# manasakani/DeviceKMC

Hardware: AMD Instinct MI355X
Metric: KMC steps/sec (higher is better)
Workload: dtype f64

## Files before the change

devicekmc_amd/csrc/common.h:

```cpp
#pragma once
#include <hip/hip_runtime.h>
#include <stdint.h>
#include <stdio.h>
#include <string.h>
#include <math.h>
#include "../../include/devicekmc_hip.h"
#include "../../include/devicekmc_hip_debug.h"

enum { DEFECT = 0, OXYGEN_DEFECT = 1, VACANCY = 2, O_EL = 3, Hf_EL = 4, Ni_EL = 5, Ti_EL = 6, Pt_EL = 7, N_EL = 8, NULL_ELEMENT = 9 };
enum { EV_GEN = 0, EV_REC = 1, EV_VDIFF = 2, EV_IDIFF = 3, EV_NULL = 4 };

#define DKMC_KB 8.617333262e-5
#define DKMC_Q 1.60217663e-19
#define DKMC_HBAR 1.054571817e-34
#define DKMC_MAX_LAYERS 5
#define WAVE 64

struct MetalSet { int n; const int *e; };

__device__ __forceinline__ bool is_metal(int el, const MetalSet &ms)
{
    bool r = false;
    for (int t = 0; t < ms.n; ++t) r |= (ms.e[t] == el);
    return r;
// ... 137 lines not shown
    double cg_tol = 1e-6;
    int current_warm_start = 1;
    int profiling = 0;
    int cb_edge_domain = 0;
    long long tcache_budget = -1;
    double pair_cut = 6.5;
    int pair_form = 0;
    int k_blocked = 1;
    int k_blocked_large = 0;
    int k_window_word_bytes = 4;
    int x_aux = 2;
    int x_slab = 1;
    int k_slab = 1;
    int x_poly = X_POLY_DEFAULT;
    int x_poly_auto = 1;
    int x_poly_rows[2] = {0, 0};
    int x_poly_form = 2;
    int x_poly1_degree = 0;
    int x_poly_form_used = 0, x_poly_products = 0;
    int x_stop_form = 2;
    double x_stop_margin = X_STOP_MARGIN_DEFAULT;
    XStopLast x_stop_last{};
    int x_slab_poly = 0;
    int x_aux_warm = 0;
    int x_items_kc = 0;
    int x_apply_form = 0;
    int x_tile_f32 = 1;
    double x_tile_drop = 0.0;
    int x_tile_drop_unit = 0;
    int x_tile_drop_auto = 1;
    long long x_tile_drop_gate = 0;
    double x_tile_drop_used = 0.0;
    int xtl_census_form = 1;
    int x_static_tiles = 2;
    int x_static_gate = 0;
    int x_static_nM = -1;
    int x_static_verify = 0;
    int x_tile_f32_fail_once = 0;
    int x_fold_form = 1;
    int x_fold_poison = 0;
    int x_nmul_form = 1;
    int x_nmul_lane_bytes = 16;
    int x_nmul_window = 2;
    int x_nmul_window_cap = 76 * 1024;
    int x_nmul_window_block = 320;
    int x_block = 16;
    int x_format = 1;
    int current_map = 0;
    int x_iter_hint = 0;
    int event_temperature = 0;
    int event_census = 0;
    int event_census_valid = 0;
    double event_census_info[16] = {0};
    dkmc_stats stats{};
    char err[512] = {0};
    int err_code = 0;
    double E_gen[DKMC_MAX_LAYERS] = {0}, E_rec[DKMC_MAX_LAYERS] = {0}, E_Vdiff[DKMC_MAX_LAYERS] = {0}, E_Odiff[DKMC_MAX_LAYERS] = {0};
    int num_layers = 0;
    static const int NBUF = 192;
    void *buf[NBUF] = {nullptr};
    size_t bufsz[NBUF] = {0};
};

constexpr int X_STATIC_GATE = 32768;
static inline int x_static_rule(int ns, int gate_override) { return ns >= (gate_override > 0 ? gate_override : X_STATIC_GATE) ? 1 : 0; }
Engine &eng();
// ... 70 lines not shown
```

devicekmc_amd/csrc/engine.hip:

```cpp
#include "common.h"
#include <stdlib.h>

int events_upload_layers();
void xstate_reset(const void *key);

static Engine g_engine;
Engine &eng() { return g_engine; }

int dkmc_fail(int code, const char *what, const char *file, int line)
{
    Engine &e = eng();
    snprintf(e.err, sizeof(e.err), "%s (%s:%d)", what, file, line);
    e.err_code = code ? code : -1;
    fprintf(stderr, "devicekmc_hip: %s\n", e.err);
    return e.err_code;
}

void *scratch(int slot, size_t bytes)
{
    Engine &e = eng();
    if (bytes == 0) bytes = 16;
    if (e.bufsz[slot] < bytes) {
        if (e.buf[slot]) { (void)hipStreamSynchronize(e.stream); (void)hipFree(e.buf[slot]); }
        size_t want = bytes + bytes / 8 + 256;
// ... 52 lines not shown
int dkmc_get_x_poly_form_used(void) { return eng().x_poly_form_used; }
int dkmc_get_x_poly_products(void) { return eng().x_poly_products; }
void dkmc_set_x_stop_form(int form) { eng().x_stop_form = form == 1 ? 1 : (form == 2 ? 2 : 0); }
int dkmc_get_x_stop_form(void) { return eng().x_stop_form; }
void dkmc_set_x_stop_margin(double kappa) { eng().x_stop_margin = (kappa > 0.0 && kappa <= 1.0) ? kappa : X_STOP_MARGIN_DEFAULT; }
double dkmc_get_x_stop_margin(void) { return eng().x_stop_margin; }
int dkmc_get_x_stop_info(int *fired, double *norm, double *rz, double *true_residual)
{
    const XStopLast &l = eng().x_stop_last;
    if (fired) *fired = l.fired;
    if (norm) *norm = l.norm;
    if (rz) *rz = l.rz;
    if (true_residual) *true_residual = l.true_res;
    return l.fired ? 0 : 1;
}
void dkmc_debug_set_x_poly1_degree(int n) { eng().x_poly1_degree = n < 0 ? 0 : (n > 20 ? 20 : n); }
void dkmc_set_x_poly_auto_rows(int n0, int n1) { Engine &e = eng(); e.x_poly_rows[0] = n0 > 0 ? n0 : 0; e.x_poly_rows[1] = n1 > e.x_poly_rows[0] ? n1 : e.x_poly_rows[0]; }
void dkmc_set_x_apply_form(int form) { eng().x_apply_form = form == 1 ? 1 : 0; }
int dkmc_get_x_apply_form(void) { return eng().x_apply_form; }
void dkmc_set_x_tile_f32(int mode) { eng().x_tile_f32 = mode == 0 ? 0 : 1; }
int dkmc_get_x_tile_f32(void) { return eng().x_tile_f32; }
void dkmc_set_x_tile_drop(double theta) { eng().x_tile_drop = theta > 0.0 ? (theta > 1e-4 ? 1e-4 : theta) : 0.0; }
double dkmc_get_x_tile_drop(void) { return eng().x_tile_drop; }
void dkmc_set_x_tile_drop_unit(int unit) { eng().x_tile_drop_unit = unit == 1 ? 1 : 0; }
int dkmc_get_x_tile_drop_unit(void) { return eng().x_tile_drop_unit; }
void dkmc_set_x_tile_drop_auto(int on) { eng().x_tile_drop_auto = on ? 1 : 0; }
int dkmc_get_x_tile_drop_auto(void) { return eng().x_tile_drop_auto; }
void dkmc_set_x_tile_drop_auto_subblocks(long long gate) { eng().x_tile_drop_gate = gate > 0 ? gate : 0; }
double dkmc_get_x_tile_drop_used(void) { return eng().x_tile_drop_used; }
void dkmc_debug_fail_true_residual_once(void) { eng().x_tile_f32_fail_once = 1; }
void dkmc_set_x_fold_form(int form) { eng().x_fold_form = form == 0 ? 0 : 1; }
int dkmc_get_x_fold_form(void) { return eng().x_fold_form; }
void dkmc_debug_poison_fold_cells(int on) { eng().x_fold_poison = on ? 1 : 0; }
void dkmc_set_x_static_tiles(int mode) { eng().x_static_tiles = (mode == 0 || mode == 1) ? mode : 2; }
int dkmc_get_x_static_tiles(void) { return eng().x_static_tiles; }
int dkmc_debug_x_static_verify(int on) { const int was = eng().x_static_verify; eng().x_static_verify = on ? 1 : 0; return was; }
void dkmc_debug_set_x_static_gate(int members) { eng().x_static_gate = members > 0 ? members : 0; }
int dkmc_x_static_rule(int members) { return x_static_rule(members, eng().x_static_gate); }
int dkmc_x_static_strips(int n_metals) { return n_metals > 0 ? n_metals / 256 : 0; }
void dkmc_set_x_nmul_form(int form) { eng().x_nmul_form = form == 0 ? 0 : 1; }
int dkmc_get_x_nmul_form(void) { return eng().x_nmul_form; }
void dkmc_set_x_nmul_lane_bytes(int bytes) { eng().x_nmul_lane_bytes = bytes == 8 ? 8 : 16; }
int dkmc_get_x_nmul_lane_bytes(void) { return eng().x_nmul_lane_bytes; }
void dkmc_set_x_nmul_window(int mode) { eng().x_nmul_window = (mode == 0 || mode == 1) ? mode : 2; }
int dkmc_get_x_nmul_window(void) { return eng().x_nmul_window; }
void dkmc_debug_set_x_nmul_window(int cap_bytes, int block_rows)
{
    Engine &e = eng();
    e.x_nmul_window_cap = cap_bytes < 0 ? 76 * 1024 : (cap_bytes > 76 * 1024 ? 76 * 1024 : cap_bytes);
    e.x_nmul_window_block = (block_rows >= 16 && block_rows <= 1024 && block_rows % 16 == 0) ? block_rows : 320;
}
void dkmc_set_x_slab(int on) { eng().x_slab = on ? 1 : 0; }
int dkmc_get_x_slab(void) { return eng().x_slab; }
void dkmc_set_x_slab_poly(int on) { eng().x_slab_poly = on ? 1 : 0; }
int dkmc_get_x_slab_poly(void) { return eng().x_slab_poly; }
void dkmc_set_x_block(int s) { eng().x_block = s < 1 ? 1 : (s > 16 ? 16 : s); }
int dkmc_get_x_block(void) { return eng().x_block; }
void dkmc_set_x_aux(int mode) { eng().x_aux = mode < 0 ? 0 : (mode > 3 ? 2 : mode); }
int dkmc_get_x_aux(void) { return eng().x_aux; }
void dkmc_set_k_blocked(int on) { eng().k_blocked = on ? 1 : 0; }
int dkmc_get_k_blocked(void) { return eng().k_blocked; }
void dkmc_set_k_blocked_large(int on) { eng().k_blocked_large = on ? 1 : 0; }
int dkmc_get_k_blocked_large(void) { return eng().k_blocked_large; }
void dkmc_set_k_window_word_bytes(int bytes) { eng().k_window_word_bytes = bytes == 2 ? 2 : 4; }
int dkmc_get_k_window_word_bytes(void) { return eng().k_window_word_bytes; }
void dkmc_set_cb_edge_domain(int atoms_only) { eng().cb_edge_domain = atoms_only ? 1 : 0; }
// ... 125 lines not shown
```

devicekmc_amd/csrc/xt.hip:

```cpp
#include "xtiles.h"
#include <hip/hip_ext.h>
int tc_prepare_tiled(const XParams &P, dkmc_gpubuf *buf, int ns, const SEntry *S, const int *aflag, const int *srank, const int *atom_site,
                     int c_lo, int c_hi, int sharded, TCacheView *out);
#include <vector>
#include <algorithm>
#include <stdlib.h>
#include <string.h>

__device__ __forceinline__ double xt_tvalue(const XParams &P, double prefac, const TCacheView &TC,
                                            double x1, double y1, double z1, double cb1, int f1, int slot1, int slotA1, int mr1,
                                            double x2, double y2, double z2, double cb2, int f2, int slot2, int slotA2, int mr2,
                                            bool have_pre = false, double pre = 0.0)
{
    const double d = site_dist(x1, y1, z1, x2, y2, z2, P.laty, P.latz, P.pbc);
    if (d < P.nn_dist) return 0.0;
    const int kind = tunnel_kind<AF_MP_VAL>(f1, f2, cb1, cb2, P.tol);
    if (!kind) return 0.0;
    if (kind == 1 && TC.enabled) {
        const bool v1 = f1 & AF_V;
        double cv;
        if (have_pre && !v1) { if (pre == pre) return -pre; }
        else if (tc_lookup(TC, v1 ? slot1 : slot2, v1 ? slotA1 : slotA2, v1 ? mr2 : mr1, cv)) return -cv;
    }
    return -wkb_T(kind, 1e-10 * d, fabs(cb1 - cb2), prefac, P.V0);
// ... 886 lines not shown

int xt_assemble_and_solve(dkmc_gpubuf *buf, const XParams &P, int ns, const SEntry *S, const int *aneigh, const int *ancnt, const int *aflag,
                          const int *srank, const int *atom_site, double *rhs, double *y, int *iters_out, double *rr_out, double *yaux, int yaux_valid, int warm)
{
    TCacheView TC{};
    Engine &e = eng(); hipStream_t st = e.stream;
    XTState &X = g_xt; X.valid = false;
    g_xlive = XLive{};
    const int Na = P.Na, Nsub = Na + 1;
    X.Nsub = Nsub; X.ns = ns;
    const int ns_pad = ((ns + XT_C - 1) / XT_C) * XT_C + XT_C;
    X.ns_pad = ns_pad;
    const int nK = (ns + XT_R - 1) / XT_R, nW = (ns + XT_C - 1) / XT_C;
    X.nK = nK; X.nW = nW;
    const long long ncell = (long long)nK * nW;
    if (ncell > 0x7ffffff0ll) return dkmc_fail(47, "update_power: too many tile cells", __FILE__, __LINE__);

    const int nbr = (Nsub + 255) / 256, m = Nsub;
    const bool sharded = comm_attached() != 0;
    const int nr = sharded ? comm_nranks() : 1, me = sharded ? comm_rank() : 0;
    int rc = 0, ntiles = 0;
    long long xs_nnz = 0;
    int *cnt = nullptr, *nsrank = nullptr, *col = nullptr, *si = nullptr, *srow = nullptr, *nitem_w = nullptr;
    xrp_t *rp = nullptr, *dpos = nullptr;
    double *val = nullptr, *sd = nullptr, *tval = nullptr, *rowpart = nullptr, *colpart = nullptr, *sc = nullptr, *r = nullptr, *p = nullptr, *t = nullptr,
           *q = nullptr, *vS = nullptr, *part = nullptr, *qS = nullptr, *sS = nullptr, *xS = nullptr, *part_pt = nullptr, *part_rr = nullptr;
    XTile *tiles = nullptr; int2 *wrange = nullptr; int *wlist = nullptr; XItem *items = nullptr; unsigned long long *d_cnt = nullptr; XCtrl *ctrl = nullptr;
    float *tval32 = nullptr;
    SNodes SN{};
    double *xbuf = nullptr;
    XStatic &K = g_xs;
    const bool k_had = K.valid;
    K.valid = false; K.pending = false; K.reused = false; K.verify_nnz = -1;
    const int nM_first = (!sharded && e.x_format != 0) ? e.x_static_nM : -1;
    const int w_static = nM_first >= 0 ? xs_w_static(nM_first) : 0;
    for (int c = 0; c < 8; ++c) K.info[c] = 0;
    for (int c = 0; c < 4; ++c) K.verify[c] = 0;
    K.info[0] = nM_first >= 0 ? 1 : 0; K.info[1] = w_static; K.info[6] = XS_NA; K.info[7] = -1;
    int t_static = 0, xs_reason = XS_NA; long long sub_static = 0;
    bool k_cand = false;
    auto assemble = [&]() -> int {
        if (g_fault_phase == 1) { g_fault_phase = 0; return dkmc_fail(90, "injected fault (assembly of X)", __FILE__, __LINE__); }
        if (sharded) { xbuf = (double *)scratch(S_CG_XCHG, ((size_t)ns * (e.x_block > 1 ? 16 : 1) + 2) * (e.x_block > 1 ? comm_nranks() : 1) * 8); if (!xbuf) return e.err_code; if (ns > 0) { rc = side_stream_init(g_side); if (rc) return rc; } }
        cnt = (int *)scratch(S_X_CNT, (size_t)(Nsub + 4) * 4);
        rp = (xrp_t *)scratch(S_X_ROWPTR, (size_t)(Nsub + 4) * sizeof(xrp_t));
        dpos = (xrp_t *)scratch(S_XT_DPOS, (size_t)(Nsub + 4) * sizeof(xrp_t));
        nsrank = (int *)scratch(S_X_SCB, (size_t)(Nsub + 4) * 4);
        if (!cnt || !rp || !dpos || !nsrank) return e.err_code;
        hipLaunchKernelGGL((k_xpat_plain<0>), dim3(nbr), dim3(256), 0, st, P, (const int *)nullptr, aneigh, ancnt, cnt, (const xrp_t *)nullptr, (int *)nullptr);
        rc = dkmc_exclusive_scan_i32_i64(cnt, rp, Nsub, rp + Nsub); if (rc) return rc;
        HIPCHK(hipMemcpyAsync(&xs_nnz, rp + Nsub, sizeof(long long), hipMemcpyDeviceToHost, st));
        HIPCHK(hipStreamSynchronize(st));
        if (xs_nnz <= 0) return dkmc_fail(10, "update_power: empty X", __FILE__, __LINE__);
        X.xs_nnz = xs_nnz;
        col = (int *)scratch(S_X_COL, (size_t)xs_nnz * 4);
        val = (double *)scratch(S_X_DATA, (size_t)xs_nnz * 8);
        if (!col || !val) return e.err_code;
        hipLaunchKernelGGL((k_xpat_plain<1>), dim3(nbr), dim3(256), 0, st, P, (const int *)nullptr, aneigh, ancnt, cnt, (const xrp_t *)rp, col);
        hipLaunchKernelGGL((k_xval<16>), dim3((Nsub + 15) / 16), dim3(256), 0, st, P, Nsub, (const SEntry *)nullptr, 0, (const int *)nullptr, (const xrp_t *)rp,
                           (const int *)col, (const double *)buf->atom_x, (const double *)buf->atom_y, (const double *)buf->atom_z, aflag,
                           (const double *)buf->atom_CB_edge, val, TCacheView{}, atom_site, dpos);
        hipLaunchKernelGGL(k_xt_node_srank, dim3(nbr), dim3(256), 0, st, Nsub, srank, nsrank);
        KCHK();
        g_xb.rp = rp; g_xb.dpos = dpos; g_xb.ci = col; g_xb.val = val; g_xb.nsrank = nsrank;
        g_xb.ax = buf->atom_x; g_xb.ay = buf->atom_y; g_xb.az = buf->atom_z;

// ... 110 lines not shown
                tval32 = (float *)scratch_try(S_XT_TVAL32, b32);
            }
            if (tval32) e.stats.x_tile_f32_bytes = (long long)b32; else e.stats.x_tile_stream = -1;
        }
        HIPCHK(hipMemsetAsync(rowpart, 0, (size_t)(ncell + 1) * XT_R * 8, st));
        HIPCHK(hipMemsetAsync(colpart, 0, (size_t)(X.nitems + 1) * XT_C * 8, st));
        HIPCHK(hipMemsetAsync(d_cnt, 0, 16, st));
        if (k_cand && (tval32 != nullptr) != K.img) { k_cand = false; xs_reason = XS_IMAGE; }
        if (w_static > 0 && !k_cand) { rc = xs_reserve(nM_first, t_static); if (rc) return rc; }
        const int t_fill0 = k_cand ? t_static : 0;
        if (nM_first < 0) {
            if (X.tile_n > 0)
                hipLaunchKernelGGL((k_xt_fill<0>), dim3(X.tile_n), dim3(XT_NT), 0, st, P, ns, (const XTile *)tiles + X.tile_lo, (int)X.sub_base, SN, TC, tval, d_cnt, tval32, 0);
        } else {
            if (t_fill0 == 0 && t_static > 0)
                hipLaunchKernelGGL((k_xt_fill<0>), dim3(t_static), dim3(XT_NT), 0, st, P, ns, (const XTile *)tiles, (int)X.sub_base, SN, TC, tval, d_cnt, tval32, t_static);
            if (X.tile_n - t_static > 0)
                hipLaunchKernelGGL((k_xt_fill<1>), dim3(X.tile_n - t_static), dim3(XT_NT), 0, st, P, ns, (const XTile *)tiles + t_static, (int)X.sub_base, SN, TC, tval, d_cnt, tval32, 0);
        }
        KCHK();
        K.info[2] = k_cand ? t_static : 0; K.info[3] = X.tile_n - t_fill0; K.info[4] = k_cand ? sub_static : 0; K.info[5] = X.sub_n - (k_cand ? sub_static : 0); K.info[6] = xs_reason;
        if (w_static > 0) {
            if (!k_cand) {
                if (t_static > 0) HIPCHK(hipMemcpyAsync(K.tiles, tiles, (size_t)t_static * sizeof(XTile), hipMemcpyDeviceToDevice, st));
                hipLaunchKernelGGL(k_xs_snapshot, dim3((nM_first + 255) / 256), dim3(256), 0, st, nM_first, SN, K.snap_d, K.snap_f);
                KCHK();
                const double par[6] = {P.tol, P.nn_dist, P.m_e, P.V0, P.laty, P.latz};
                memcpy(K.par, par, sizeof(par)); K.pbc = P.pbc;
                K.key = (const void *)buf->site_x; K.nM = nM_first; K.w_static = w_static; K.t_static = t_static; K.sub_static = sub_static;
            }
            K.tval = e.buf[S_XT_TVAL]; K.tval_cap = e.bufsz[S_XT_TVAL]; K.img = tval32 != nullptr;
            K.tval32 = K.img ? e.buf[S_XT_TVAL32] : nullptr; K.tval32_cap = K.img ? e.bufsz[S_XT_TVAL32] : 0;
            K.pending = true; K.reused = k_cand;
        }
        if (e.x_static_verify && nM_first >= 0 && ncell > 0) {
            rc = xs_verify(P, ns, nK, nW, ncell, SN, TC, cmask, tiles, ntiles, X.nsub_total, tval, tval32); if (rc) return rc;
        }
        g_xb.tval32 = tval32;
        g_xb.tval = tval; g_xb.rowpart = rowpart; g_xb.colpart = colpart;
        X.valid = true;

        sc = (double *)scratch(S_CG_S, (size_t)m * 8); r = (double *)scratch(S_CG_R, (size_t)m * 8);
        p = (double *)scratch(S_CG_P, (size_t)m * 8); t = (double *)scratch(S_CG_T, (size_t)m * 8);
        q = (double *)scratch(S_XT_Q, (size_t)m * 8);
        vS = (double *)scratch(S_CG_PS, (size_t)ns_pad * 3 * 8);
        part = (double *)scratch(S_CG_PART, (size_t)3 * 8192 * 8);
        ctrl = (XCtrl *)scratch(S_CG_CTRL, sizeof(XCtrl));
        if (!sc || !r || !p || !t || !q || !vS || !part || !ctrl) return e.err_code;
        qS = vS; sS = vS + ns_pad; xS = vS + 2 * (size_t)ns_pad;
        HIPCHK(hipMemsetAsync(vS, 0, (size_t)ns_pad * 3 * 8, st));
        part_pt = part; part_rr = part + 4096;
        return 0;
    };
    rc = assemble();
    if (sharded) rc = comm_agree(rc, "assembly of X");
    if (rc) return rc;

    const double tol2 = e.cg_tol * e.cg_tol;

    if (ns > 0) {
        hipLaunchKernelGGL(k_xt_fill_f64, dim3((ns + 255) / 256), dim3(256), 0, st, qS, (long long)ns, 1.0);
        rc = xt_tile_sums<0>(qS, xS, 1); if (rc) return rc;
    }
    hipLaunchKernelGGL(k_xt_scale_init, dim3(nbr), dim3(256), 0, st, m, (const xrp_t *)dpos, val, (const int *)nsrank, (const double *)xS, sc, rhs, y, q, sS, qS);
    KCHK();

// ... 484 lines not shown
```

devicekmc_amd/csrc/xt_live.h:

```cpp
#pragma once

XLive g_xlive;

constexpr double XTL_DROP_AUTO_THETA = 1e-10;
constexpr long long XTL_DROP_GATE = 246272;
double xtl_drop_rule(long long stored_subblocks, long long gate_override)
{
    const long long gate = gate_override > 0 ? gate_override : XTL_DROP_GATE;
    return stored_subblocks > 0 && stored_subblocks >= gate ? XTL_DROP_AUTO_THETA : 0.0;
}
extern "C" double dkmc_xtl_drop_rule(long long stored_subblocks) { return xtl_drop_rule(stored_subblocks, eng().x_tile_drop_gate); }

__global__ __launch_bounds__(XT_NT) void k_xtl_census(int nK, const XTile *__restrict__ tiles, int sub_base, const double *__restrict__ tval,
                                                      const double *__restrict__ sS, double theta, int unit, unsigned *__restrict__ lcmask,
                                                      int *__restrict__ tflag, unsigned long long *__restrict__ cnt)
{
    __shared__ double rs[XT_R], mx[XT_C / XT_SBW];
    const XTile td = tiles[blockIdx.x];
    const int tid = threadIdx.x, q = tid >> 5, c = tid & 31;
    if (tid < XT_R) rs[tid] = sS[XT_R * td.k + tid];
    __syncthreads();
    double m = 0.0;
    if ((td.mask >> q) & 1u) {
        const int sl = __popc(td.mask & ((1u << q) - 1u));
// ... 44 lines not shown
            const int r0 = 8 * (it >> 1) + 2 * (it & 1) + (l >> 4);
            const double ra = rs[r0], rb = rs[r0 + 4];
            one(v.x, ra, s0); one(v.y, ra, s1); one(v.z, rb, s0); one(v.w, rb, s1);
        }
    }
#pragma unroll
    for (int off = 16; off > 0; off >>= 1) { up = fmax(up, __shfl_xor(up, off, WAVE)); lo = fmax(lo, __shfl_xor(lo, off, WAVE)); }
    const bool dead = up * (1.0 + BAND) < theta, sure = lo * (1.0 - BAND) >= theta;
    const bool again = present && !dead && !sure;
    double m = 0.0;
    if (again) {
        const double *src = tval + slot * XT_SUB + l;
        const double scc = sS[XT_C * td.w + XT_SBW * q + l];
#pragma unroll 8
        for (int r = 0; r < XT_R; ++r) m = fmax(m, (rs[r] * fabs(src[r * XT_SBW])) * scc);
    }
#pragma unroll
    for (int off = 16; off > 0; off >>= 1) m = fmax(m, __shfl_xor(m, off, WAVE));
    const bool lives = again ? m >= theta : (present && sure);
    if (l == 0) lvq[q] = again ? (lives ? 2 : -1) : (lives ? 1 : 0);
    __syncthreads();
    if (tid == 0) {
        int own = 0, re = 0; unsigned lm = 0u;
#pragma unroll
        for (int u = 0; u < XT_C / XT_SBW; ++u) { if (lvq[u] > 0) { ++own; lm |= 1u << u; } if (lvq[u] == 2 || lvq[u] == -1) ++re; }
        const bool live = own > 0;
        lcmask[(size_t)td.w * nK + td.k] = live ? (unit == 1 ? lm : td.mask) : 0u;
        tflag[blockIdx.x] = live ? 1 : 0;
        if (live) { atomicAdd(cnt, 1ull); atomicAdd(cnt + 1, (unsigned long long)__popc(td.mask)); }
        if (own) atomicAdd(cnt + 2, (unsigned long long)own);
        if (re) atomicAdd(cnt + 3, (unsigned long long)re);
    }
}
__global__ __launch_bounds__(XT_NT) void k_xtl_compact(int nK, const XTile *__restrict__ tiles, int sub_base, const unsigned *__restrict__ lcmask,
                                                       const int *__restrict__ lsoff, const float4 *__restrict__ src32, float4 *__restrict__ dst32)
{
    const XTile td = tiles[blockIdx.x];
    const size_t ci = (size_t)td.w * nK + td.k;
    const unsigned lm = lcmask[ci] & td.mask;
    if (!lm) return;
    const float4 *s = src32 + (size_t)(td.soff - sub_base) * (XT_SUB / 4) + threadIdx.x;
    float4 *d = dst32 + (size_t)lsoff[ci] * (XT_SUB / 4) + threadIdx.x;
    int dl = 0;
#pragma unroll
    for (int q = 0; q < XT_C / XT_SBW; ++q)
        if ((lm >> q) & 1u) { d[(size_t)dl * (XT_SUB / 4)] = s[(size_t)__popc(td.mask & ((1u << q) - 1u)) * (XT_SUB / 4)]; ++dl; }
}
__global__ __launch_bounds__(XT_NT) void k_xtl_zero_dead(long long n, int per, int nW, const XTile *__restrict__ tiles, const int *__restrict__ tflag,
                                                         double *__restrict__ rowpartB)
{
    const long long i = (long long)blockIdx.x * blockDim.x + threadIdx.x;
    if (i >= n) return;
    const int t = (int)(i / per);
    if (tflag[t]) return;
    const XTile td = tiles[t];
    rowpartB[((size_t)td.k * nW + td.w) * per + (size_t)(i % per)] = 0.0;
}

static hipEvent_t g_xl_ev[3]; static bool g_xl_ev_ready = false;

static long long g_xtl_reread = 0;
static int xt_live_census(double theta, int unit, const double *sS, unsigned **lcmask_out, int **tflag_out, unsigned long long *h4)
{
    Engine &e = eng(); hipStream_t st = e.stream; const XTState &X = g_xt;
    const long long ncell = (long long)X.nK * X.nW;
    unsigned *lcmask = (unsigned *)scratch(S_XTL_CELLS, (size_t)(ncell + 4) * 4 * 3);
    int *tflag = (int *)scratch(S_XTL_TFLAG, (size_t)(X.ntiles + 8) * 4 + 32);
    if (!lcmask || !tflag) return e.err_code;
    unsigned long long *cnt = reinterpret_cast<unsigned long long *>(tflag + ((X.ntiles + 7) & ~7));
    HIPCHK(hipMemsetAsync(lcmask, 0, (size_t)(ncell + 4) * 4, st));
    HIPCHK(hipMemsetAsync(cnt, 0, 32, st));
    if (e.xtl_census_form == 1 && g_xb.tval32 && theta >= 1e-290)
        hipLaunchKernelGGL(k_xtl_census_img, dim3(X.ntiles), dim3(XT_NT), 0, st, X.nK, (const XTile *)g_xb.tiles, (int)X.sub_base, (const double *)g_xb.tval,
                           reinterpret_cast<const float4 *>(g_xb.tval32), sS, theta, unit, lcmask, tflag, cnt);
    else
        hipLaunchKernelGGL(k_xtl_census, dim3(X.ntiles), dim3(XT_NT), 0, st, X.nK, (const XTile *)g_xb.tiles, (int)X.sub_base, (const double *)g_xb.tval, sS, theta,
                           unit, lcmask, tflag, cnt);
    KCHK();
    HIPCHK(hipMemcpyAsync(h4, cnt, 32, hipMemcpyDeviceToHost, st));
    HIPCHK(hipStreamSynchronize(st));
    g_xtl_reread = (long long)h4[3];
    *lcmask_out = lcmask; *tflag_out = tflag;
    return 0;
}
extern "C" int dkmc_debug_xtl_census_form(int form) { const int was = eng().xtl_census_form; eng().xtl_census_form = form == 1 ? 1 : 0; return was; }
extern "C" long long dkmc_debug_xtl_census_reread(void) { return g_xtl_reread; }

int xt_live_build(double theta, int unit, const double *sS, XLive *lv)
{
    Engine &e = eng(); hipStream_t st = e.stream; const XTState &X = g_xt;
    *lv = XLive{};
    if (!(theta > 0.0) || !X.valid || comm_attached() || X.tile_n != X.ntiles || X.ntiles <= 0 || !g_xb.tval32 || !sS) return 0;
    const bool prof = e.profiling != 0;
    if (prof && !g_xl_ev_ready) { for (auto &ev : g_xl_ev) HIPCHK(hipEventCreate(&ev)); g_xl_ev_ready = true; }
    if (prof) HIPCHK(hipEventRecord(g_xl_ev[0], st));
    const int nK = X.nK, nW = X.nW;
    const long long ncell = (long long)nK * nW;
    unsigned *lcmask = nullptr; int *tflag = nullptr; unsigned long long h3[4] = {0, 0, 0, 0};
    if (int rc = xt_live_census(theta, unit, sS, &lcmask, &tflag, h3)) return rc;
    lv->tflag = tflag;
    lv->info[1] = X.ntiles; lv->info[2] = (long long)h3[0]; lv->info[3] = X.nsub_total; lv->info[4] = (long long)h3[1]; lv->info[5] = (long long)h3[2];
    const int nlive = (int)h3[0]; const long long nsub_live = (long long)h3[unit == 1 ? 2 : 1];
    if ((X.nsub_total - nsub_live) * 64 < X.nsub_total) { lv->state = -2; return 0; }
    int *ltoff = (int *)lcmask + (ncell + 4), *lsoff = ltoff + (ncell + 4);
    hipLaunchKernelGGL(k_xt_cell_counts, dim3((unsigned)((ncell + 255) / 256)), dim3(256), 0, st, ncell, (const unsigned *)lcmask, ltoff, lsoff);
    if (int rc = dkmc_exclusive_scan_i32(ltoff, ltoff, (int)ncell, ltoff + ncell)) return rc;
    if (int rc = dkmc_exclusive_scan_i32(lsoff, lsoff, (int)ncell, lsoff + ncell)) return rc;
    if (prof) HIPCHK(hipEventRecord(g_xl_ev[1], st));
    const size_t bytes = (size_t)(nsub_live + 4) * XT_SUB * 4;
    float *c32 = (float *)scratch_try(S_XTL_TVAL32, bytes);
    if (!c32) { lv->state = -1; return 0; }
    XTile *ltiles = (XTile *)scratch(S_XTL_TILES, (size_t)(nlive + 1) * sizeof(XTile));
    int2 *lwrange = (int2 *)scratch(S_XTL_WRANGE, (size_t)(nK + 4) * sizeof(int2));
    int *lwlist = (int *)scratch(S_XTL_WLIST, ((size_t)nK * (nW + 1) + 4) * sizeof(int));
    if (!ltiles || !lwrange || !lwlist) return e.err_code;
    hipLaunchKernelGGL(k_xtl_compact, dim3(X.ntiles), dim3(XT_NT), 0, st, nK, (const XTile *)g_xb.tiles, (int)X.sub_base, (const unsigned *)lcmask, (const int *)lsoff,
                       reinterpret_cast<const float4 *>(g_xb.tval32), reinterpret_cast<float4 *>(c32));
    hipLaunchKernelGGL(k_xt_tile_list, dim3((unsigned)((ncell + 255) / 256)), dim3(256), 0, st, nK, ncell, (const unsigned *)lcmask, (const int *)ltoff, (const int *)lsoff, ltiles);
    hipLaunchKernelGGL(k_xt_wrange, dim3((nK + 255) / 256), dim3(256), 0, st, nK, nW, (const unsigned *)lcmask, lwrange, lwlist);
    KCHK();
    XShare sh{};
    if (int rc = xt_build_items(nK, nW, X.kc, nlive, nsub_live, ltoff, ltiles, 1, 0, S_XTL_NITEMW, S_XTL_ITEMS, S_XTL_SPLIT, &sh, 2)) return rc;
    if ((sh.item_lo | sh.item_n) & 3) return dkmc_fail(48, "live view: run list not padded to groups of four", __FILE__, __LINE__);
    if (prof) {
        HIPCHK(hipEventRecord(g_xl_ev[2], st));
        HIPCHK(hipEventSynchronize(g_xl_ev[2]));
        float ms = 0.f;
        HIPCHK(hipEventElapsedTime(&ms, g_xl_ev[0], g_xl_ev[1])); lv->ms[0] = ms;
        HIPCHK(hipEventElapsedTime(&ms, g_xl_ev[1], g_xl_ev[2])); lv->ms[1] = ms;
    }
    lv->tiles = ltiles; lv->items = sh.items ? sh.items + sh.item_lo : nullptr; lv->item_n = sh.item_n; lv->wrange = lwrange; lv->wlist = lwlist; lv->nitem_w = sh.nitem_w;
    lv->nrecords = sh.nitems >> sh.rec_shift; lv->nitems = sh.nitems; lv->tval32 = c32;
// ... 74 lines not shown
```

devicekmc_amd/lib.py:

```python
import ctypes as C
import os

_HERE = os.path.dirname(os.path.abspath(__file__))
LIB_PATH = os.path.join(_HERE, "libdevicekmc_hip.so")

c_int_p = C.POINTER(C.c_int)
c_dbl_p = C.POINTER(C.c_double)
vp = C.c_void_p


class dkmc_gpubuf(C.Structure):
    _PTRS = ["site_charge", "site_power", "site_potential_boundary", "site_potential_charge", "site_temperature",
             "site_CB_edge", "T_bg", "atom_power", "atom_CB_edge", "atom_virtual_potentials", "atom_charge",
             "site_element", "atom_element", "site_x", "site_y", "site_z", "atom_x", "atom_y", "atom_z",
             "metal_types", "sigma", "k", "lattice", "freq", "neigh_idx", "site_layer",
             "Device_row_ptr_d", "Device_col_indices_d", "contact_left_row_ptr", "contact_left_col_indices",
             "contact_right_row_ptr", "contact_right_col_indices"]
    _INTS = ["Device_nnz", "contact_left_nnz", "contact_right_nnz", "num_metal_types_", "N_", "nn_", "N_atom_"]
    _fields_ = [(n, vp) for n in _PTRS] + [(n, C.c_int) for n in _INTS]


class dkmc_stats(C.Structure):
    _fields_ = [("cg_iters_K", C.c_int), ("cg_iters_CB", C.c_int), ("cg_iters_X", C.c_int),
                ("cg_rr_K", C.c_double), ("cg_rr_CB", C.c_double), ("cg_rr_X", C.c_double),
# ... 44 lines not shown
    "dkmc_set_x_poly_auto_rows": (None, [_I, _I]),
    "dkmc_set_x_poly_form": (None, [_I]),
    "dkmc_get_x_poly_form": (_I, []),
    "dkmc_get_x_poly_form_used": (_I, []),
    "dkmc_get_x_poly_products": (_I, []),
    "dkmc_debug_set_x_poly1_degree": (None, [_I]),
    "dkmc_set_x_stop_form": (None, [_I]),
    "dkmc_get_x_stop_form": (_I, []),
    "dkmc_set_x_stop_margin": (None, [_D]),
    "dkmc_get_x_stop_margin": (_D, []),
    "dkmc_get_x_stop_info": (_I, [c_int_p, c_dbl_p, c_dbl_p, c_dbl_p]),
    "dkmc_debug_get_x_stop_rt0": (_I, [_I, vp]),
    "dkmc_xtb_stop_rule": (_I, [_I]),
    "dkmc_set_x_tile_f32": (None, [_I]),
    "dkmc_get_x_tile_f32": (_I, []),
    "dkmc_set_x_tile_drop": (None, [_D]),
    "dkmc_get_x_tile_drop": (_D, []),
    "dkmc_set_x_tile_drop_unit": (None, [_I]),
    "dkmc_get_x_tile_drop_unit": (_I, []),
    "dkmc_set_x_tile_drop_auto": (None, [_I]),
    "dkmc_get_x_tile_drop_auto": (_I, []),
    "dkmc_get_x_tile_drop_used": (_D, []),
    "dkmc_get_x_tile_live_info": (_I, [C.POINTER(C.c_longlong), c_dbl_p]),
    "dkmc_xt_get_live": (_I, [_D, vp, vp]),
    "dkmc_xt_get_live_masks": (_I, [_D, vp]),
    "dkmc_debug_fail_true_residual_once": (None, []),
    "dkmc_set_x_fold_form": (None, [_I]),
    "dkmc_get_x_fold_form": (_I, []),
    "dkmc_debug_poison_fold_cells": (None, [_I]),
    "dkmc_xt_get_fold_lists": (_I, [_I, c_int_p, c_int_p, vp]),
    "dkmc_set_x_static_tiles": (None, [_I]),
    "dkmc_get_x_static_tiles": (_I, []),
    "dkmc_get_x_static_info": (_I, [C.POINTER(C.c_longlong)]),
    "dkmc_debug_x_static_verify": (_I, [_I]),
    "dkmc_debug_get_x_static_verify": (_I, [C.POINTER(C.c_longlong)]),
    "dkmc_x_static_strips": (_I, [_I]),
    "dkmc_x_static_rule": (_I, [_I]),
    "dkmc_debug_set_x_static_gate": (None, [_I]),
    "dkmc_xt_get_srow": (_I, [c_int_p, vp]),
    "dkmc_xt_get_diag": (_I, [vp]),
    "dkmc_set_x_nmul_form": (None, [_I]),
    "dkmc_get_x_nmul_form": (_I, []),
    "dkmc_set_x_nmul_lane_bytes": (None, [_I]),
    "dkmc_get_x_nmul_lane_bytes": (_I, []),
    "dkmc_set_x_nmul_window": (None, [_I]),
    "dkmc_get_x_nmul_window": (_I, []),
    "dkmc_debug_set_x_nmul_window": (None, [_I, _I]),
    "dkmc_set_x_apply_form": (None, [_I]),
    "dkmc_get_x_apply_form": (_I, []),
    "dkmc_set_x_slab": (None, [_I]),
    "dkmc_get_x_slab": (_I, []),
    "dkmc_set_x_slab_poly": (None, [_I]),
    "dkmc_get_x_slab_poly": (_I, []),
    "dkmc_set_x_aux_warm": (None, [_I]),
    "dkmc_get_x_aux_warm": (_I, []),
    "dkmc_set_x_aux": (None, [_I]),
    "dkmc_get_x_aux": (_I, []),
    "dkmc_set_k_blocked": (None, [_I]),
    "dkmc_get_k_blocked": (_I, []),
    "dkmc_set_k_blocked_large": (None, [_I]),
    "dkmc_get_k_blocked_large": (_I, []),
    "dkmc_set_k_window_word_bytes": (None, [_I]),
    "dkmc_get_k_window_word_bytes": (_I, []),
    "dkmc_kcg_form_info": (_I, [C.POINTER(dkmc_gpubuf), C.POINTER(C.c_longlong)]),
    "dkmc_kcg_form_words": (_I, [C.POINTER(dkmc_gpubuf), C.POINTER(C.c_longlong)]),
    "dkmc_debug_k_system": (_I, [C.POINTER(dkmc_gpubuf), _I, _I, _I, _I, _D, _D, _D, _D, _I, vp, vp, vp, vp]),
# ... 169 lines not shown
```

include/devicekmc_hip.h:

```cpp
#ifndef DEVICEKMC_HIP_H
#define DEVICEKMC_HIP_H

#ifdef __cplusplus
extern "C" {
#endif

#ifndef DKMC_ELEMENT_T
#define DKMC_ELEMENT_T int
#endif
typedef struct dkmc_gpubuf {
    int *site_charge;
    double *site_power, *site_potential_boundary, *site_potential_charge, *site_temperature;
    double *site_CB_edge;
    double *T_bg;
    double *atom_power;
    double *atom_CB_edge;
    double *atom_virtual_potentials;
    int *atom_charge;
    DKMC_ELEMENT_T *site_element;
    DKMC_ELEMENT_T *atom_element;
    double *site_x, *site_y, *site_z;
    double *atom_x, *atom_y, *atom_z;
    DKMC_ELEMENT_T *metal_types;
    double *sigma, *k, *lattice, *freq;
// ... 57 lines not shown
void dkmc_set_pair_cutoff(double x_cut);
void dkmc_reset_pair_sum_cache(void);
void dkmc_set_pair_form(int form);
int dkmc_get_pair_form(void);
void dkmc_set_x_block(int s);
int dkmc_get_x_block(void);
void dkmc_set_x_poly(int degree);
int dkmc_get_x_poly(void);
void dkmc_set_x_poly_auto(int on);
int dkmc_get_x_poly_auto(void);
void dkmc_set_x_poly_form(int form);
int dkmc_get_x_poly_form(void);
int dkmc_get_x_poly_form_used(void);
int dkmc_get_x_poly_products(void);
void dkmc_set_x_stop_form(int form);
int dkmc_get_x_stop_form(void);
void dkmc_set_x_stop_margin(double kappa);
double dkmc_get_x_stop_margin(void);
int dkmc_get_x_stop_info(int *fired, double *norm, double *rz, double *true_residual);
void dkmc_set_x_nmul_form(int form);
int dkmc_get_x_nmul_form(void);
void dkmc_set_x_tile_f32(int mode);
int dkmc_get_x_tile_f32(void);
void dkmc_set_x_tile_drop(double theta);
double dkmc_get_x_tile_drop(void);
void dkmc_set_x_tile_drop_unit(int unit);
int dkmc_get_x_tile_drop_unit(void);
void dkmc_set_x_tile_drop_auto(int on);
int dkmc_get_x_tile_drop_auto(void);
double dkmc_get_x_tile_drop_used(void);
void dkmc_set_x_static_tiles(int mode);
int dkmc_get_x_static_tiles(void);
int dkmc_get_x_static_info(long long *info8);
void dkmc_set_x_nmul_lane_bytes(int bytes);
int dkmc_get_x_nmul_lane_bytes(void);
void dkmc_set_x_nmul_window(int mode);
int dkmc_get_x_nmul_window(void);
void dkmc_set_x_slab(int on);
int dkmc_get_x_slab(void);
void dkmc_set_x_slab_poly(int on);
int dkmc_get_x_slab_poly(void);
void dkmc_set_k_slab(int on);
int dkmc_get_k_slab(void);
void dkmc_set_x_aux(int mode);
int dkmc_get_x_aux(void);
void dkmc_set_x_aux_warm(int on);
int dkmc_get_x_aux_warm(void);
void dkmc_set_k_blocked(int on);
int dkmc_get_k_blocked(void);
void dkmc_set_k_blocked_large(int on);
int dkmc_get_k_blocked_large(void);
void dkmc_set_k_window_word_bytes(int bytes);
int dkmc_get_k_window_word_bytes(void);
void dkmc_set_current_warm_start(int mode);
int dkmc_get_current_warm_start(void);
int dkmc_get_current_warm_vector(const dkmc_gpubuf *buf, double *h_out, int capacity, int *n_out);
int dkmc_set_current_warm_vector(const dkmc_gpubuf *buf, const double *h_in, int n);
int dkmc_get_current_warm_aux(const dkmc_gpubuf *buf, double *h_out, long long capacity, long long *n_out);
int dkmc_set_current_warm_aux(const dkmc_gpubuf *buf, const double *h_in, long long n);
void dkmc_set_profiling(int on);
void dkmc_set_x_format(int tiled);
int dkmc_get_x_format(void);

int dkmc_gpubuf_create(dkmc_gpubuf *buf, int N, int N_atom, int nn, int num_metal_types,
                       const int *h_site_layer, const double *h_site_x, const double *h_site_y,
                       const double *h_site_z, const int *h_neigh_idx, const int *h_metals,
// ... 162 lines not shown
```

include/devicekmc_hip_debug.h:

```cpp
#ifndef DEVICEKMC_HIP_DEBUG_H
#define DEVICEKMC_HIP_DEBUG_H
#include "devicekmc_hip.h"
#ifdef __cplusplus
extern "C" {
#endif

int dkmc_xt_time_share(int nranks, int rank, int reps, double *apply_us, double *side_us , int *items_out, long long *subblocks_out);
int dkmc_xt_check_shares(int nranks, double *max_abs_diff, double *max_abs, long long *subblocks_sum, long long *items_sum, int *items_total);
int dkmc_xtb_check_product(int width, double *max_abs_diff, double *max_abs);
int dkmc_xtb_poly_coeffs(int degree, double *pc);
int dkmc_xtb_poly_rule(int m);
void dkmc_set_x_poly_auto_rows(int n0, int n1);
int dkmc_xtb_test_nstep(int m, const long long *rp, const int *ci, const double *val, const double *sc, const double *in, const double *add,
                        double ca, double cb, int form, const int *rowlist, int nlist, const int *nsrank, int ns, double *out, double *qs);
int dkmc_xtb_check_poly(int degree, int form, const double *in, double *out, double *qs);
void dkmc_debug_set_x_nmul_window(int cap_bytes, int block_rows);
int dkmc_xtb_time_poly(int degree, int reps, double *us);
typedef struct dkmc_xtb_ctrl { double rr[2]; int done_local, sharded; int done; int iters; int abort_local, aborted; int pad[2]; int xchg_timeout, pad2; } dkmc_xtb_ctrl;
int dkmc_xtb_test_gram(int m, const double *P, const double *T, const double *R, const int *nsrank, int ns, int ng, int done_word, double *gfin,
                       dkmc_xtb_ctrl *ctrl_out);
int dkmc_xtb_test_small(int it, int s, int nrg, const double *gblocks, double tol2, const dkmc_xtb_ctrl *ctrl_in, double *mats, dkmc_xtb_ctrl *ctrl_out);
int dkmc_xtb_test_step(int m, int it, const double *mats, int done_word, double *y0, double *R, double *P, const double *T, const double *sc,
                       const int *nsrank, int ns, const int *rowlist, int nlist, double *Ypanel, double *qs);
int dkmc_xtb_poly1_coeffs(int n, double *pc, double *qmin);
void dkmc_debug_set_x_poly1_degree(int n);
int dkmc_xtb_test_gram1(int m, const double *const *panels, int ng, int done_word, double *gfin);
int dkmc_xtb_test_step1(int m, int it, const double *mats, int done_word, double *y0, double *const *panels, const double *sc, const int *nsrank, int ns,
                        double *qs);
int dkmc_xtb_test_step1_norm(int m, int it, const double *mats, int done_word, double *y0, double *const *panels, const double *sc, const int *nsrank, int ns,
                             double *qs, double bound2, double rr_in, double *rec3, dkmc_xtb_ctrl *ctrl_out);
int dkmc_debug_get_x_stop_rt0(int m, double *rt0);
int dkmc_xtb_stop_rule(int m);
int dkmc_xtb_time_apply(int width, int variant, int reps, double *us);
int dkmc_xt_tile_census(long long *hist);
void dkmc_set_x_items(int kc);
void dkmc_debug_fail_true_residual_once(void);
int dkmc_xtb_tile_product(int width, int stored_bytes, double *out);
int dkmc_xt_get_tiles(long long *ntiles, long long *nsub, int *tiles4, double *tval);
int dkmc_xtb_time_apply_stored(int width, int stored_bytes, int reps, double *us);
int dkmc_get_x_tile_live_info(long long *info8, double *ms2);
int dkmc_debug_xtl_census_form(int form);
long long dkmc_debug_xtl_census_reread(void);
double dkmc_xtl_drop_rule(long long stored_subblocks);
void dkmc_set_x_tile_drop_auto_subblocks(long long gate);
int dkmc_xt_get_live(double theta, int *live_per_tile, double *sS_out);
int dkmc_xt_get_live_masks(double theta, int *mask_per_tile);
void dkmc_set_x_fold_form(int form);
int dkmc_get_x_fold_form(void);
void dkmc_debug_poison_fold_cells(int on);
int dkmc_xt_get_fold_lists(int live, int *nK, int *nW, int *rows);
int dkmc_debug_x_static_verify(int on);
int dkmc_debug_get_x_static_verify(long long *v4);
int dkmc_x_static_strips(int n_metals);
int dkmc_x_static_rule(int members);
void dkmc_debug_set_x_static_gate(int members);
int dkmc_xt_get_srow(int *ns_out, int *srow_out);
int dkmc_xt_get_diag(double *d_out);
void dkmc_set_x_apply_form(int form);
int dkmc_get_x_apply_form(void);
void dkmc_debug_inject_fault(int phase, int iteration);
int dkmc_debug_step_stop_word(int m, int it, int done_word, int *updated, int *done_after);

int dkmc_xtb_emulate_slabs(int nranks, int width, double tol, int time_rank, int sweep_cap, double *rel_diff, int *iters_slab, int *iters_ref,
                           double *times_us, long long *xdoubles, int *rows_min_max);

int dkmc_xtb_slab_last(int *exchanges_per_sweep, long long *halo_doubles_per_exchange, double *nmul_us);

int dkmc_kcg_emulate_slabs(dkmc_gpubuf *buf, int N, int N_left, int N_right, double Vd, double high_G, double low_G, int num_metals, int nranks, int time_rank,
                           int iter_cap, double *max_abs_diff, int *iters_slab, int *iters_ref, double *times_us, long long *halo_rows);

int dkmc_kcg_form_info(dkmc_gpubuf *buf, long long *info );
int dkmc_kcg_form_words(dkmc_gpubuf *buf, long long *info );
int dkmc_debug_k_system(dkmc_gpubuf *buf, int rule, int N, int N_left, int N_right, double VL, double VR, double high_G, double low_G, int num_metals,
                        const double *v_site, double *t_site, double *diag_site, double *rhs_site);
int dkmc_debug_kbw_halfword_pos(int width, int entry);
void dkmc_debug_kbw_segment_cap(int cap);
// ... 23 lines not shown
```

Baseline: 6.093.

## Cache per-subblock max summaries for kept static tiles to shortcut live census

Adds a summary kernel that, for each stored static-tile subblock, records the largest absolute value and its row and column. The summary is rebuilt only when the static tile values change. A new census kernel uses these summaries to decide, from a cheap exact element and an upper bound, whether a kept subblock is live, and falls back to the float32 and then float64 scan only when the bounds disagree. The census counters are spread over 64 cache lines to reduce atomic contention. The cost is an extra summary buffer, one extra kernel launch when tiles are rebuilt, and a larger host copy of the counters.

```diff
diff --git a/devicekmc_amd/csrc/common.h b/devicekmc_amd/csrc/common.h
--- a/devicekmc_amd/csrc/common.h
+++ b/devicekmc_amd/csrc/common.h
@@ -193,6 +193,7 @@
     long long x_tile_drop_gate = 0;
     double x_tile_drop_used = 0.0;
     int xtl_census_form = 1;
+    int x_census_form = 1;
     int x_static_tiles = 2;
     int x_static_gate = 0;
     int x_static_nM = -1;
diff --git a/devicekmc_amd/csrc/engine.hip b/devicekmc_amd/csrc/engine.hip
--- a/devicekmc_amd/csrc/engine.hip
+++ b/devicekmc_amd/csrc/engine.hip
@@ -108,6 +108,8 @@
 void dkmc_set_x_fold_form(int form) { eng().x_fold_form = form == 0 ? 0 : 1; }
 int dkmc_get_x_fold_form(void) { return eng().x_fold_form; }
 void dkmc_debug_poison_fold_cells(int on) { eng().x_fold_poison = on ? 1 : 0; }
+void dkmc_set_x_census_form(int form) { eng().x_census_form = form == 0 ? 0 : 1; }
+int dkmc_get_x_census_form(void) { return eng().x_census_form; }
 void dkmc_set_x_static_tiles(int mode) { eng().x_static_tiles = (mode == 0 || mode == 1) ? mode : 2; }
 int dkmc_get_x_static_tiles(void) { return eng().x_static_tiles; }
 int dkmc_debug_x_static_verify(int on) { const int was = eng().x_static_verify; eng().x_static_verify = on ? 1 : 0; return was; }
diff --git a/devicekmc_amd/csrc/xt.hip b/devicekmc_amd/csrc/xt.hip
--- a/devicekmc_amd/csrc/xt.hip
+++ b/devicekmc_amd/csrc/xt.hip
@@ -942,6 +942,7 @@
     XStatic &K = g_xs;
     const bool k_had = K.valid;
     K.valid = false; K.pending = false; K.reused = false; K.verify_nnz = -1;
+    g_xks.live = false;
     const int nM_first = (!sharded && e.x_format != 0) ? e.x_static_nM : -1;
     const int w_static = nM_first >= 0 ? xs_w_static(nM_first) : 0;
     for (int c = 0; c < 8; ++c) K.info[c] = 0;
@@ -1118,6 +1119,11 @@
             K.tval = e.buf[S_XT_TVAL]; K.tval_cap = e.bufsz[S_XT_TVAL]; K.img = tval32 != nullptr;
             K.tval32 = K.img ? e.buf[S_XT_TVAL32] : nullptr; K.tval32_cap = K.img ? e.bufsz[S_XT_TVAL32] : 0;
             K.pending = true; K.reused = k_cand;
+        }
+        if (!k_cand) g_xks.have = false;
+        if (w_static > 0 && e.x_census_form == 1 && tval32 && sub_static > 0 && X.sub_base == 0 && X.tile_n == ntiles) {
+            if (!(g_xks.have && g_xks.n == sub_static && g_xks.t == t_static && g_xks.tval == (const void *)tval)) { rc = xt_kept_summarise(tval, t_static, sub_static); if (rc) return rc; }
+            g_xks.live = true;
         }
         if (e.x_static_verify && nM_first >= 0 && ncell > 0) {
             rc = xs_verify(P, ns, nK, nW, ncell, SN, TC, cmask, tiles, ntiles, X.nsub_total, tval, tval32); if (rc) return rc;
diff --git a/devicekmc_amd/csrc/xt_live.h b/devicekmc_amd/csrc/xt_live.h
--- a/devicekmc_amd/csrc/xt_live.h
+++ b/devicekmc_amd/csrc/xt_live.h
@@ -100,6 +100,133 @@
         if (re) atomicAdd(cnt + 3, (unsigned long long)re);
     }
 }
+constexpr int XTL_CNT_LINES = 64;
+struct __attribute__((aligned(16))) XSum { double vmax; int r, c; };
+struct XKeptSum {
+    XSum *d = nullptr; size_t cap = 0;
+    long long n = 0; int t = 0; const void *tval = nullptr;
+    bool have = false;
+    bool live = false;
+};
+static XKeptSum g_xks;
+
+__global__ __launch_bounds__(XT_NT) void k_xtl_summary(long long nsub, const double *__restrict__ tval, XSum *__restrict__ out)
+{
+    const long long sb = (long long)blockIdx.x * (XT_NT / 32) + (threadIdx.x >> 5);
+    const int l = threadIdx.x & 31;
+    double m = -1.0; int r = 0, c = l;
+    if (sb < nsub) {
+        const double *src = tval + (size_t)sb * XT_SUB + l;
+#pragma unroll 8
+        for (int i = 0; i < XT_R; ++i) { const double a = fabs(src[i * XT_SBW]); if (a > m) { m = a; r = i; } }
+    }
+#pragma unroll
+    for (int off = 16; off > 0; off >>= 1) {
+        const double om = __shfl_xor(m, off, WAVE); const int orr = __shfl_xor(r, off, WAVE), oc = __shfl_xor(c, off, WAVE);
+        if (om > m || (om == m && oc < c)) { m = om; r = orr; c = oc; }
+    }
+    if (sb < nsub && l == 0) { XSum s; s.vmax = m > 0.0 ? m : 0.0; s.r = r; s.c = c; out[sb] = s; }
+}
+static int xt_kept_summarise(const double *tval, int ntile, long long nsub)
+{
+    XKeptSum &Q = g_xks;
+    Q.have = false;
+    if (Q.cap < (size_t)nsub) {
+        if (Q.d) (void)hipFree(Q.d);
+        Q.d = nullptr; Q.cap = 0;
+        const size_t cap = (size_t)nsub + (size_t)nsub / 8 + 16;
+        HIPCHK(hipMalloc((void **)&Q.d, cap * sizeof(XSum)));
+        Q.cap = cap;
+    }
+    hipLaunchKernelGGL(k_xtl_summary, dim3((unsigned)((nsub + XT_NT / 32 - 1) / (XT_NT / 32))), dim3(XT_NT), 0, eng().stream, nsub, tval, Q.d);
+    KCHK();
+    Q.n = nsub; Q.t = ntile; Q.tval = (const void *)tval; Q.have = true;
+    return 0;
+}
+
+__global__ __launch_bounds__(XT_NT) void k_xtl_census_sum(int nK, const XTile *__restrict__ tiles, int sub_base, const double *__restrict__ tval,
+                                                          const float4 *__restrict__ tval32, const double *__restrict__ sS, double theta, int unit,
+                                                          int t_kept, const XSum *__restrict__ summ,
+                                                          unsigned *__restrict__ lcmask, int *__restrict__ tflag, unsigned long long *__restrict__ cnt)
+{
+    constexpr double BAND = 1.0 / 4194304.0, FMIN = 1.1754943508222875e-38, FMAX = 3.4028234663852886e+38;
+    __shared__ double rs[XT_R]; __shared__ int lvq[XT_C / XT_SBW], kq[XT_C / XT_SBW];
+    const XTile td = tiles[blockIdx.x];
+    const int tid = threadIdx.x, q = tid >> 5, l = tid & 31;
+    if (tid < XT_R) rs[tid] = sS[XT_R * td.k + tid];
+    __syncthreads();
+    const bool present = (td.mask >> q) & 1u;
+    const size_t slot = (size_t)(td.soff - sub_base) + __popc(td.mask & ((1u << q) - 1u));
+    const bool kept = present && (int)blockIdx.x < t_kept;
+    bool decided = false, sum_live = false;
+    if ((int)blockIdx.x < t_kept) {
+        double mr = rs[l], ms = sS[XT_C * td.w + XT_SBW * q + l];
+#pragma unroll
+        for (int off = 16; off > 0; off >>= 1) { mr = fmax(mr, __shfl_xor(mr, off, WAVE)); ms = fmax(ms, __shfl_xor(ms, off, WAVE)); }
+        if (present) {
+            const XSum s = summ[slot];
+            const double es = (rs[s.r & (XT_R - 1)] * s.vmax) * sS[XT_C * td.w + XT_SBW * q + (s.c & (XT_SBW - 1))];
+            const double ub = (mr * s.vmax) * ms;
+            sum_live = es >= theta;
+            decided = sum_live || ub < theta;
+        }
+    }
+    const bool rd = present && !decided;
+    double up = 0.0, lo = 0.0;
+    if (rd) {
+        const float4 *src = tval32 + slot * (XT_SUB / 4) + l;
+        const double s0 = sS[XT_C * td.w + XT_SBW * q + 2 * (l & 15)], s1 = sS[XT_C * td.w + XT_SBW * q + 2 * (l & 15) + 1];
+        auto one = [&](float v, double r, double sc) {
+            const double a = fabs((double)v);
+            const double p = (r * fmax(a, FMIN)) * sc;
+            up = fmax(up, p);
+            lo = fmax(lo, (a >= FMIN && a <= FMAX) ? p : 0.0);
+        };
+#pragma unroll
+        for (int it = 0; it < 8; ++it) {
+            const float4 v = src[it * 32];
+            const int r0 = 8 * (it >> 1) + 2 * (it & 1) + (l >> 4);
+            const double ra = rs[r0], rb = rs[r0 + 4];
+            one(v.x, ra, s0); one(v.y, ra, s1); one(v.z, rb, s0); one(v.w, rb, s1);
+        }
+    }
+#pragma unroll
+    for (int off = 16; off > 0; off >>= 1) { up = fmax(up, __shfl_xor(up, off, WAVE)); lo = fmax(lo, __shfl_xor(lo, off, WAVE)); }
+    const bool dead = up * (1.0 + BAND) < theta, sure = lo * (1.0 - BAND) >= theta;
+    const bool again = rd && !dead && !sure;
+    double m = 0.0;
+    if (again) {
+        const double *src = tval + slot * XT_SUB + l;
+        const double scc = sS[XT_C * td.w + XT_SBW * q + l];
+#pragma unroll 8
+        for (int r = 0; r < XT_R; ++r) m = fmax(m, (rs[r] * fabs(src[r * XT_SBW])) * scc);
+    }
+#pragma unroll
+    for (int off = 16; off > 0; off >>= 1) m = fmax(m, __shfl_xor(m, off, WAVE));
+    const bool lives = decided ? sum_live : (again ? m >= theta : (rd && sure));
+    if (l == 0) {
+        lvq[q] = again ? (lives ? 2 : -1) : (lives ? 1 : 0);
+        kq[q] = kept ? (decided ? (sum_live ? 1 : 0) : 2) : 0;
+    }
+    __syncthreads();
+    if (tid == 0) {
+        int own = 0, re = 0, kl = 0, kr = 0; unsigned lm = 0u;
+#pragma unroll
+        for (int u = 0; u < XT_C / XT_SBW; ++u) {
+            if (lvq[u] > 0) { ++own; lm |= 1u << u; }
+            if (lvq[u] == 2 || lvq[u] == -1) ++re;
+            kl += kq[u] == 1 ? 1 : 0; kr += kq[u] == 2 ? 1 : 0;
+        }
+        const bool live = own > 0;
+        lcmask[(size_t)td.w * nK + td.k] = live ? (unit == 1 ? lm : td.mask) : 0u;
+        tflag[blockIdx.x] = live ? 1 : 0;
+        unsigned long long *c8 = cnt + 8 * (blockIdx.x & (XTL_CNT_LINES - 1));
+        if (live) { atomicAdd(c8, 1ull); atomicAdd(c8 + 1, (unsigned long long)__popc(td.mask)); }
+        if (own) atomicAdd(c8 + 2, (unsigned long long)own);
+        if (re) atomicAdd(c8 + 3, (unsigned long long)re);
+        if (kl | kr) atomicAdd(c8 + 4, (unsigned long long)kl | ((unsigned long long)kr << 32));
+    }
+}
 __global__ __launch_bounds__(XT_NT) void k_xtl_compact(int nK, const XTile *__restrict__ tiles, int sub_base, const unsigned *__restrict__ lcmask,
                                                        const int *__restrict__ lsoff, const float4 *__restrict__ src32, float4 *__restrict__ dst32)
 {
@@ -128,31 +255,64 @@
 static hipEvent_t g_xl_ev[3]; static bool g_xl_ev_ready = false;
 
 static long long g_xtl_reread = 0;
+static long long g_xtl_kept[4] = {0, 0, 0, 0}, g_xtl_kept_solve[4] = {0, 0, 0, 0};
 static int xt_live_census(double theta, int unit, const double *sS, unsigned **lcmask_out, int **tflag_out, unsigned long long *h4)
 {
     Engine &e = eng(); hipStream_t st = e.stream; const XTState &X = g_xt;
     const long long ncell = (long long)X.nK * X.nW;
     unsigned *lcmask = (unsigned *)scratch(S_XTL_CELLS, (size_t)(ncell + 4) * 4 * 3);
-    int *tflag = (int *)scratch(S_XTL_TFLAG, (size_t)(X.ntiles + 8) * 4 + 32);
+    int *tflag = (int *)scratch(S_XTL_TFLAG, (size_t)(X.ntiles + 8) * 4 + 64 * XTL_CNT_LINES);
     if (!lcmask || !tflag) return e.err_code;
     unsigned long long *cnt = reinterpret_cast<unsigned long long *>(tflag + ((X.ntiles + 7) & ~7));
+    unsigned long long h8[8] = {0, 0, 0, 0, 0, 0, 0, 0}, hl[8 * XTL_CNT_LINES];
     HIPCHK(hipMemsetAsync(lcmask, 0, (size_t)(ncell + 4) * 4, st));
-    HIPCHK(hipMemsetAsync(cnt, 0, 32, st));
-    if (e.xtl_census_form == 1 && g_xb.tval32 && theta >= 1e-290)
+    HIPCHK(hipMemsetAsync(cnt, 0, 64 * XTL_CNT_LINES, st));
+    const bool img = e.xtl_census_form == 1 && g_xb.tval32 && theta >= 1e-290;
+    long long n_kept = -1;
+    if (img && e.x_census_form == 1) {
+        const XKeptSum &Q = g_xks;
+        const bool sum = Q.live && Q.have && Q.d && Q.tval == (const void *)g_xb.tval && X.sub_base == 0 && Q.t <= X.ntiles && Q.n <= X.nsub_total;
+        n_kept = sum ? Q.n : 0;
+        hipLaunchKernelGGL(k_xtl_census_sum, dim3(X.ntiles), dim3(XT_NT), 0, st, X.nK, (const XTile *)g_xb.tiles, (int)X.sub_base, (const double *)g_xb.tval,
+                           reinterpret_cast<const float4 *>(g_xb.tval32), sS, theta, unit, sum ? Q.t : 0, (const XSum *)Q.d, lcmask, tflag, cnt);
+    } else if (img)
         hipLaunchKernelGGL(k_xtl_census_img, dim3(X.ntiles), dim3(XT_NT), 0, st, X.nK, (const XTile *)g_xb.tiles, (int)X.sub_base, (const double *)g_xb.tval,
                            reinterpret_cast<const float4 *>(g_xb.tval32), sS, theta, unit, lcmask, tflag, cnt);
     else
         hipLaunchKernelGGL(k_xtl_census, dim3(X.ntiles), dim3(XT_NT), 0, st, X.nK, (const XTile *)g_xb.tiles, (int)X.sub_base, (const double *)g_xb.tval, sS, theta,
                            unit, lcmask, tflag, cnt);
     KCHK();
-    HIPCHK(hipMemcpyAsync(h4, cnt, 32, hipMemcpyDeviceToHost, st));
+    HIPCHK(hipMemcpyAsync(hl, cnt, 64 * XTL_CNT_LINES, hipMemcpyDeviceToHost, st));
     HIPCHK(hipStreamSynchronize(st));
+    for (int i = 0; i < 8 * XTL_CNT_LINES; ++i) h8[i & 7] += hl[i];
+    for (int c = 0; c < 4; ++c) { h4[c] = h8[c]; g_xtl_kept[c] = 0; }
+    if (n_kept >= 0) {
+        g_xtl_kept[0] = (long long)(h8[4] & 0xffffffffull); g_xtl_kept[2] = (long long)(h8[4] >> 32);
+        g_xtl_kept[1] = n_kept - g_xtl_kept[0] - g_xtl_kept[2]; g_xtl_kept[3] = X.nsub_total - n_kept;
+    }
     g_xtl_reread = (long long)h4[3];
     *lcmask_out = lcmask; *tflag_out = tflag;
     return 0;
 }
 extern "C" int dkmc_debug_xtl_census_form(int form) { const int was = eng().xtl_census_form; eng().xtl_census_form = form == 1 ? 1 : 0; return was; }
 extern "C" long long dkmc_debug_xtl_census_reread(void) { return g_xtl_reread; }
+extern "C" int dkmc_get_x_census_info(long long *info8)
+{
+    if (info8) for (int c = 0; c < 4; ++c) { info8[c] = g_xtl_kept_solve[c]; info8[4 + c] = g_xtl_kept[c]; }
+    return 0;
+}
+extern "C" int dkmc_debug_get_x_census_kept(long long *n, double *vmax, int *rc)
+{
+    Engine &e = eng(); const XKeptSum &Q = g_xks;
+    const bool sum = g_xt.valid && Q.live && Q.have && Q.d && Q.tval == (const void *)g_xb.tval;
+    if (n) *n = sum ? Q.n : 0;
+    if (!sum || (!vmax && !rc)) return 0;
+    std::vector<XSum> h((size_t)Q.n);
+    HIPCHK(hipStreamSynchronize(e.stream));
+    HIPCHK(hipMemcpy(h.data(), Q.d, (size_t)Q.n * sizeof(XSum), hipMemcpyDeviceToHost));
+    for (long long i = 0; i < Q.n; ++i) { if (vmax) vmax[i] = h[i].vmax; if (rc) { rc[2 * i] = h[i].r; rc[2 * i + 1] = h[i].c; } }
+    return 0;
+}
 
 int xt_live_build(double theta, int unit, const double *sS, XLive *lv)
 {
@@ -166,6 +326,7 @@
     const long long ncell = (long long)nK * nW;
     unsigned *lcmask = nullptr; int *tflag = nullptr; unsigned long long h3[4] = {0, 0, 0, 0};
     if (int rc = xt_live_census(theta, unit, sS, &lcmask, &tflag, h3)) return rc;
+    for (int c = 0; c < 4; ++c) g_xtl_kept_solve[c] = g_xtl_kept[c];
     lv->tflag = tflag;
     lv->info[1] = X.ntiles; lv->info[2] = (long long)h3[0]; lv->info[3] = X.nsub_total; lv->info[4] = (long long)h3[1]; lv->info[5] = (long long)h3[2];
     const int nlive = (int)h3[0]; const long long nsub_live = (long long)h3[unit == 1 ? 2 : 1];
diff --git a/devicekmc_amd/lib.py b/devicekmc_amd/lib.py
--- a/devicekmc_amd/lib.py
+++ b/devicekmc_amd/lib.py
@@ -100,6 +100,10 @@
     "dkmc_set_x_static_tiles": (None, [_I]),
     "dkmc_get_x_static_tiles": (_I, []),
     "dkmc_get_x_static_info": (_I, [C.POINTER(C.c_longlong)]),
+    "dkmc_set_x_census_form": (None, [_I]),
+    "dkmc_get_x_census_form": (_I, []),
+    "dkmc_get_x_census_info": (_I, [C.POINTER(C.c_longlong)]),
+    "dkmc_debug_get_x_census_kept": (_I, [C.POINTER(C.c_longlong), vp, vp]),
     "dkmc_debug_x_static_verify": (_I, [_I]),
     "dkmc_debug_get_x_static_verify": (_I, [C.POINTER(C.c_longlong)]),
     "dkmc_x_static_strips": (_I, [_I]),
diff --git a/include/devicekmc_hip.h b/include/devicekmc_hip.h
--- a/include/devicekmc_hip.h
+++ b/include/devicekmc_hip.h
@@ -113,6 +113,9 @@
 void dkmc_set_x_static_tiles(int mode);
 int dkmc_get_x_static_tiles(void);
 int dkmc_get_x_static_info(long long *info8);
+void dkmc_set_x_census_form(int form);
+int dkmc_get_x_census_form(void);
+int dkmc_get_x_census_info(long long *info8);
 void dkmc_set_x_nmul_lane_bytes(int bytes);
 int dkmc_get_x_nmul_lane_bytes(void);
 void dkmc_set_x_nmul_window(int mode);
diff --git a/include/devicekmc_hip_debug.h b/include/devicekmc_hip_debug.h
--- a/include/devicekmc_hip_debug.h
+++ b/include/devicekmc_hip_debug.h
@@ -42,6 +42,7 @@
 int dkmc_debug_xtl_census_form(int form);
 long long dkmc_debug_xtl_census_reread(void);
 double dkmc_xtl_drop_rule(long long stored_subblocks);
+int dkmc_debug_get_x_census_kept(long long *n, double *vmax, int *rc);
 void dkmc_set_x_tile_drop_auto_subblocks(long long gate);
 int dkmc_xt_get_live(double theta, int *live_per_tile, double *sS_out);
 int dkmc_xt_get_live_masks(double theta, int *mask_per_tile);
```

New measurement: 6.150 (median of 6 runs). About the same (+0.9%).
